# li779/mitsuba-im

Hardware: AMD Instinct MI355X
Metric: Msamples/sec at 1920x1080 path-trace, max depth 8 (higher is better)
Workload: dtype f32; 1 GPU; C2: Cornell box (synthetic, 32 triangles), 1920x1080, sobol sampler, 256 spp (256 per GPU-share), maxDepth 8, rrDepth 5, box filter, 1xMI355X wavefront path tracer per GPU; one process per GPU, rows interleaved over the ranks, RCCL film reduce; parallelism=tiles1, face=C-ABI (mi_render_run)

## Files before the change

### mitsuba-im_amd/csrc/kernels_trace.hip

```cpp
#include "kernels_common.h"
#include <algorithm>
#include "trace.h"
#include "trace_fused.h"

template <int STACK, int AN, bool WIDE>
__global__ __launch_bounds__(WG) void k_extend(DScene sc, Queues q, int buf) {
    __shared__ int s_stk[(STACK > 0 ? STACK : 1) * WG];
    __shared__ f4 s_exact[STACK > 0 ? 1 : MI_PACKET_MAX * 3];
    const uint32_t tid = threadIdx.x;
    unsigned long long rays = 0;
    if (STACK == 0) packetStage(sc, s_exact);
    for (uint32_t seg = blockIdx.x; seg < q.n_seg; seg += gridDim.x) {
    const uint32_t n = q.count[buf][seg];
    const uint64_t segBase = (uint64_t) seg * q.cap;
    rays += n;
    for (uint32_t i = tid; i < n; i += WG) {
        float4 ro = q.rayO[buf][segBase + i], rd = q.rayD[buf][segBase + i];
        v3 o = V(ro.x, ro.y, ro.z), d = V(rd.x, rd.y, rd.z);
        float mint, maxt, t = 0, u = 0, v = 0; uint32_t prim = 0xFFFFFFFFu; bool hit = false; int inst = -1;
        if (clipInterval(sc, o, d, ro.w, rd.w, false, mint, maxt)) {
            if (STACK == 0) hit = packetIntersect<false, AN>(sc, (AS<true>::p4) s_exact, o, d, mint, maxt, t, prim, u, v);
            else hit = traverse<false, AN, WIDE>(sc, o, d, mint, maxt, s_stk + tid, t, prim, u, v, inst);
        }
        q.hit[segBase + i] = make_float4(t, u, v, __uint_as_float(hit ? prim : 0xFFFFFFFFu));
        if ((AN & 2) && q.hitInst) q.hitInst[segBase + i] = inst;
    }
    }
    if (tid == 0 && rays) atomicAdd(&q.counters[0], rays);
}

template <int STACK, int AN, bool WIDE>
__global__ __launch_bounds__(WG) void k_shadow(DScene sc, Queues q) {
    __shared__ int s_stk[(STACK > 0 ? STACK : 1) * WG];
    __shared__ f4 s_exact[STACK > 0 ? 1 : MI_PACKET_MAX * 3];
    const uint32_t tid = threadIdx.x;
    if (STACK == 0) packetStage(sc, s_exact);
    for (uint32_t seg = blockIdx.x; seg < q.n_seg; seg += gridDim.x) {
    const uint32_t n = q.shCount[seg];
    const uint64_t segBase = (uint64_t) seg * q.cap;
    for (uint32_t i = tid; i < n; i += WG) {
        float4 so = q.shO[segBase + i], sd = q.shD[segBase + i];
        v3 o = V(so.x, so.y, so.z), d = V(sd.x, sd.y, sd.z);
        float mint, maxt, t, u, v; uint32_t prim; bool occluded = false; int inst;
        if (clipInterval(sc, o, d, MI_EPSILON, so.w, true, mint, maxt)) {
            if (STACK == 0) occluded = packetIntersect<true, AN>(sc, (AS<true>::p4) s_exact, o, d, mint, maxt, t, prim, u, v);
            else occluded = traverse<true, AN, WIDE>(sc, o, d, mint, maxt, s_stk + tid, t, prim, u, v, inst);
        }
        if (!occluded) {
            float4 c = q.shC[segBase + i]; const uint32_t pid = __float_as_uint(sd.w);
            float4 a = q.acc[pid]; a.x += c.x; a.y += c.y; a.z += c.z; q.acc[pid] = a;
        }
    }
    }
}



template <bool WIDE>
__global__ __launch_bounds__(WG) void k_extend_f(DScene sc, Queues q, int buf, uint32_t *ticket, uint32_t thr) {
    __shared__ int s_lds[FZ_LDS_WORDS];
    fusedStage<false, WIDE>(sc, q, buf, ticket, thr, s_lds);
}
template <bool WIDE>
__global__ __launch_bounds__(WG) void k_shadow_f(DScene sc, Queues q, uint32_t *ticket, uint32_t thr) {
    __shared__ int s_lds[FZ_LDS_WORDS];
    fusedStage<true, WIDE>(sc, q, 0, ticket, thr, s_lds);
}

template <bool ANY, bool WIDE, int LS>
__global__ __launch_bounds__(WG) void k_debug_fused(DScene sc, Queues q, uint32_t *ticket, uint32_t thr, int *maxSp) {
    __shared__ int s_lds[(LS + 10) * WG];
    fusedStage<ANY, WIDE, LS, true>(sc, q, 0, ticket, thr, s_lds, maxSp);
}

__global__ __launch_bounds__(WG) void k_debug_intersect(DScene sc, const float *rays, uint64_t n, int anyHit, float *out, int *outInst) {
    __shared__ int s_stk[STACK_DEPTH * WG];
    __shared__ f4 s_exact[MI_PACKET_MAX * 3];
    if (sc.packet_n) packetStage(sc, s_exact);
    const uint64_t i = (uint64_t) blockIdx.x * WG + threadIdx.x;
    if (i >= n) return;
    const float *r = rays + i * 8;
    v3 o = V(r[0], r[1], r[2]), d = V(r[4], r[5], r[6]);
    float mint, maxt, t = 0, u = 0, v = 0; uint32_t prim = 0xFFFFFFFFu; bool hit = false; int inst = -1;
    if (clipInterval(sc, o, d, r[3], r[7], anyHit != 0, mint, maxt)) {
        if (sc.packet_n) { if (anyHit) hit = packetIntersect<true, 1>(sc, (AS<true>::p4) s_exact, o, d, mint, maxt, t, prim, u, v); else hit = packetIntersect<false, 1>(sc, (AS<true>::p4) s_exact, o, d, mint, maxt, t, prim, u, v); }
        else if (sc.bvh_wide) { if (anyHit) hit = traverse<true, 3, true>(sc, o, d, mint, maxt, s_stk + threadIdx.x, t, prim, u, v, inst); else hit = traverse<false, 3, true>(sc, o, d, mint, maxt, s_stk + threadIdx.x, t, prim, u, v, inst); }
        else if (anyHit) hit = traverse<true, 3, false>(sc, o, d, mint, maxt, s_stk + threadIdx.x, t, prim, u, v, inst);
        else hit = traverse<false, 3, false>(sc, o, d, mint, maxt, s_stk + threadIdx.x, t, prim, u, v, inst);
    }
    if (outInst) outInst[i] = hit ? inst : -1;
    out[i * 4] = t; out[i * 4 + 1] = u; out[i * 4 + 2] = v; out[i * 4 + 3] = hit ? (anyHit ? 1.0f : (float) prim) : -1.0f;
}

__global__ __launch_bounds__(WG) void k_ray_intersect(DScene sc, const float *rays, uint64_t n, mi_intersection *out) {
    __shared__ int s_stk[STACK_DEPTH * WG];
    __shared__ f4 s_exact[MI_PACKET_MAX * 3];
    if (sc.packet_n) packetStage(sc, s_exact);
    const uint64_t i = (uint64_t) blockIdx.x * WG + threadIdx.x;
    if (i >= n) return;
    const float *r = rays + i * 8;
    v3 o = V(r[0], r[1], r[2]), d = V(r[4], r[5], r[6]);
    float mint, maxt, t = 0, u = 0, v = 0; uint32_t prim = 0xFFFFFFFFu; bool hit = false; int inst = -1;
    if (clipInterval(sc, o, d, r[3], r[7], false, mint, maxt)) {
        if (sc.packet_n) hit = packetIntersect<false, 1>(sc, (AS<true>::p4) s_exact, o, d, mint, maxt, t, prim, u, v);
        else if (sc.bvh_wide) hit = traverse<false, 3, true>(sc, o, d, mint, maxt, s_stk + threadIdx.x, t, prim, u, v, inst);
        else hit = traverse<false, 3, false>(sc, o, d, mint, maxt, s_stk + threadIdx.x, t, prim, u, v, inst);
    }
    mi_intersection rec; memset(&rec, 0, sizeof(rec)); rec.valid = hit ? 1u : 0u; rec.prim = 0xFFFFFFFFu; rec.instance = -1; rec.material = -1; rec.emitter = -1;
    if (hit) {
        Tabs<false> tb; tb.shade4 = (AS<false>::p4) sc.shade; tb.materials4 = (AS<false>::p4) sc.materials; tb.emitters4 = (AS<false>::p4) sc.emitters; tb.emitter_cdf = sc.emitter_cdf; tb.area_cdf = sc.area_cdf;
        Hit h;
        if (inst >= 0) fillHitInstanced(sc, tb, sc.instances[inst], o, d, t, prim, u, v, h);
        else if (prim >= sc.n_tris) fillHitAnalytic(sc.analytic[prim - sc.n_tris], o, d, t, u, v, h);
        else fillHit<false, true>(sc, tb, d, t, prim, u, v, h);
        if (inst < 0 && prim >= sc.n_tris) { v3 du, dv; analyticUV(sc.analytic[prim - sc.n_tris], u, v, o + d * t, h.uvx, h.uvy, du, dv); }
        rec.t = t; rec.p[0] = h.p.x; rec.p[1] = h.p.y; rec.p[2] = h.p.z; rec.ng[0] = h.ng.x; rec.ng[1] = h.ng.y; rec.ng[2] = h.ng.z;
        rec.ns[0] = h.ns.x; rec.ns[1] = h.ns.y; rec.ns[2] = h.ns.z; rec.s[0] = h.s.x; rec.s[1] = h.s.y; rec.s[2] = h.s.z; rec.tt[0] = h.t.x; rec.tt[1] = h.t.y; rec.tt[2] = h.t.z;
        rec.uv[0] = h.uvx; rec.uv[1] = h.uvy; rec.wi[0] = h.wi.x; rec.wi[1] = h.wi.y; rec.wi[2] = h.wi.z; rec.bary[0] = u; rec.bary[1] = v;
        rec.prim = prim; rec.instance = inst; rec.material = h.material; rec.emitter = h.emitter;
    }
    out[i] = rec;
}

extern "C" {
static const bool kForceStack24 = getenv("MI355PT_STACK24") != nullptr;
#define MI_BY_STACK_W(KERNEL, AN, W, ...) do { \
    if (sc.bvh_depth <= 8) hipLaunchKernelGGL((KERNEL<8, AN, W>), dim3(grid), dim3(WG), 0, st, __VA_ARGS__); \
    else if (sc.bvh_depth <= 12) hipLaunchKernelGGL((KERNEL<12, AN, W>), dim3(grid), dim3(WG), 0, st, __VA_ARGS__); \
    else if (sc.bvh_depth <= 16) hipLaunchKernelGGL((KERNEL<16, AN, W>), dim3(grid), dim3(WG), 0, st, __VA_ARGS__); \
    else if (sc.bvh_depth <= 20 && !kForceStack24) hipLaunchKernelGGL((KERNEL<20, AN, W>), dim3(grid), dim3(WG), 0, st, __VA_ARGS__); \
    else if (sc.bvh_depth <= 24) hipLaunchKernelGGL((KERNEL<24, AN, W>), dim3(grid), dim3(WG), 0, st, __VA_ARGS__); \
    else if (sc.bvh_depth <= 28) hipLaunchKernelGGL((KERNEL<28, AN, W>), dim3(grid), dim3(WG), 0, st, __VA_ARGS__); \
    else hipLaunchKernelGGL((KERNEL<STACK_DEPTH, AN, W>), dim3(grid), dim3(WG), 0, st, __VA_ARGS__); } while (0)
#define MI_BY_STACK(KERNEL, AN, ...) do { \
    if (sc.packet_n) hipLaunchKernelGGL((KERNEL<0, (AN) & 1, false>), dim3(grid), dim3(WG), 0, st, __VA_ARGS__); \
    else if (sc.bvh_wide) MI_BY_STACK_W(KERNEL, AN, true, __VA_ARGS__); \
    else MI_BY_STACK_W(KERNEL, AN, false, __VA_ARGS__); } while (0)
void mi_launch_extend(const DScene &sc, const Queues &q, int buf, uint32_t grid, hipStream_t st) {
    const int mode = (sc.n_analytic ? 1 : 0) | (sc.n_instances ? 2 : 0);
    if (mode == 3) MI_BY_STACK(k_extend, 3, sc, q, buf); else if (mode == 2) MI_BY_STACK(k_extend, 2, sc, q, buf); else if (mode == 1) MI_BY_STACK(k_extend, 1, sc, q, buf); else MI_BY_STACK(k_extend, 0, sc, q, buf);
}
void mi_launch_shadow(const DScene &sc, const Queues &q, uint32_t grid, hipStream_t st) {
    const int mode = (sc.n_analytic ? 1 : 0) | (sc.n_instances ? 2 : 0);
    if (mode == 3) MI_BY_STACK(k_shadow, 3, sc, q); else if (mode == 2) MI_BY_STACK(k_shadow, 2, sc, q); else if (mode == 1) MI_BY_STACK(k_shadow, 1, sc, q); else MI_BY_STACK(k_shadow, 0, sc, q);
}
#undef MI_BY_STACK
#undef MI_BY_STACK_W
static const int kFused = [] { const char *e = getenv("MI355PT_FUSED"); return e && e[0] ? atoi(e) : 1; }();
static const uint32_t kFusedThr = [] { const char *e = getenv("MI355PT_FUSED_THR"); const int v = e && e[0] ? atoi(e) : 48; return (uint32_t) (v < 1 ? 1 : (v > 64 ? 64 : v)); }();
static const uint32_t kFusedGrid = [] { const char *e = getenv("MI355PT_FUSED_GRID"); const int v = e && e[0] ? atoi(e) : 1792; return (uint32_t) (v < 1 ? 1 : (v > 16384 ? 16384 : v)); }();
bool mi_fused_walk(const DScene &sc) { return kFused && (sc.bvh_wide || kFused == 2) && !sc.packet_n && !sc.n_analytic && !sc.n_instances && sc.geo_bytes < 0xFFFFFF00ull; }
uint32_t mi_fused_grid(void) { return kFusedGrid; }
void mi_launch_extend_fused(const DScene &sc, const Queues &q, int buf, uint32_t *ticket, hipStream_t st) {
    const uint32_t g = kFusedGrid;
    if (sc.bvh_wide) hipLaunchKernelGGL((k_extend_f<true>), dim3(g), dim3(WG), 0, st, sc, q, buf, ticket, kFusedThr); else hipLaunchKernelGGL((k_extend_f<false>), dim3(g), dim3(WG), 0, st, sc, q, buf, ticket, kFusedThr);
}
void mi_launch_shadow_fused(const DScene &sc, const Queues &q, uint32_t *ticket, hipStream_t st) {
    const uint32_t g = kFusedGrid;
    if (sc.bvh_wide) hipLaunchKernelGGL((k_shadow_f<true>), dim3(g), dim3(WG), 0, st, sc, q, ticket, kFusedThr); else hipLaunchKernelGGL((k_shadow_f<false>), dim3(g), dim3(WG), 0, st, sc, q, ticket, kFusedThr);
}
void mi_launch_debug_fused(const DScene &sc, const Queues &q, int anyHit, uint32_t ldsStack, uint32_t *ticket, uint32_t thr, uint32_t grid, int *maxSp, hipStream_t st) {
#define MI_DBG_FUSED(ANY, WIDE) do { \
    if (ldsStack == 4u) hipLaunchKernelGGL((k_debug_fused<ANY, WIDE, 4>), dim3(grid), dim3(WG), 0, st, sc, q, ticket, thr, maxSp); \
    else hipLaunchKernelGGL((k_debug_fused<ANY, WIDE, FZ_LDS_STACK>), dim3(grid), dim3(WG), 0, st, sc, q, ticket, thr, maxSp); } while (0)
    if (anyHit) { if (sc.bvh_wide) MI_DBG_FUSED(true, true); else MI_DBG_FUSED(true, false); }
    else { if (sc.bvh_wide) MI_DBG_FUSED(false, true); else MI_DBG_FUSED(false, false); }
#undef MI_DBG_FUSED
}
uint32_t mi_fused_lds_stack(void) { return FZ_LDS_STACK; }
void mi_launch_ray_intersect(const DScene &sc, const float *rays, uint64_t n, mi_intersection *out, hipStream_t st) { hipLaunchKernelGGL(k_ray_intersect, dim3((unsigned) ((n + WG - 1) / WG)), dim3(WG), 0, st, sc, rays, n, out); }
void mi_launch_debug_intersect(const DScene &sc, const float *rays, uint64_t n, int anyHit, float *out, int *outInst, hipStream_t st) { hipLaunchKernelGGL(k_debug_intersect, dim3((unsigned) ((n + WG - 1) / WG)), dim3(WG), 0, st, sc, rays, n, anyHit, out, outInst); }
}
```

### mitsuba-im_amd/csrc/scene_build.cpp

```cpp
#include "scene_host.h"
#include <algorithm>
#include <cmath>
#include <cstdlib>
#include <cstring>
#include <limits>

namespace mi {

struct V3 { float x, y, z; };
static inline V3 mk(float x, float y, float z) { return V3{x, y, z}; }
static inline V3 operator+(V3 a, V3 b) { return mk(a.x + b.x, a.y + b.y, a.z + b.z); }
static inline V3 operator-(V3 a, V3 b) { return mk(a.x - b.x, a.y - b.y, a.z - b.z); }
static inline V3 operator*(V3 a, float s) { return mk(a.x * s, a.y * s, a.z * s); }
static inline float dot(V3 a, V3 b) { return a.x * b.x + a.y * b.y + a.z * b.z; }
static inline V3 cross(V3 a, V3 b) { return mk(a.y * b.z - a.z * b.y, a.z * b.x - a.x * b.z, a.x * b.y - a.y * b.x); }
static inline float comp(V3 a, int i) { return i == 0 ? a.x : (i == 1 ? a.y : a.z); }
static inline V3 normalize(V3 a) { float inv = 1.0f / std::sqrt(dot(a, a)); return a * inv; }
static inline V3 vmin(V3 a, V3 b) { return mk(std::min(a.x, b.x), std::min(a.y, b.y), std::min(a.z, b.z)); }
static inline V3 vmax(V3 a, V3 b) { return mk(std::max(a.x, b.x), std::max(a.y, b.y), std::max(a.z, b.z)); }

static void triaccelLoad(TriAccelD &ta, V3 A, V3 B, V3 C) {
    static const int wald[4] = {1, 2, 0, 1};
    V3 b = C - A, c = B - A, N = cross(c, b);
    int k = 0;
// ... 301 lines not shown
                            int ql = (int) std::floor(((double) comp(k.lo, a) - o) / step), qh = (int) std::ceil(((double) comp(k.hi, a) - o) / step);
                            ql = std::min(std::max(ql, 0), 255); qh = std::min(std::max(qh, 0), 255);
                            while (ql > 0 && (float) ((float) o + (float) ql * (float) step) > comp(k.lo, a)) --ql;
                            while (qh < 255 && (float) ((float) o + (float) qh * (float) step) < comp(k.hi, a)) ++qh;
                            w.qlo[a] |= (uint32_t) ql << (8 * c); w.qhi[a] |= (uint32_t) qh << (8 * c);
                        }
                        if (k.count > 0) w.child[c] = leafCode(triBase + k.first, k.count);
                        else { int need = 0, needD = 0; w.child[c] = run(kids[c], need, needD); sub = std::max(sub, need); subD = std::max(subD, needD); }
                    }
                    std::memcpy(&nodes[dev], &w, sizeof(w));
                    need = sub + 1;
                    needD = subD + 3;
                    return dev;
                } };
            Emit em{nodes, bld, triBase, emptyChild, area}; int need = 0, needD = 0; const int dev = em.run(root, need, needD); treeNeed.push_back(need + 1); treeNeedDirect.push_back(needD + 1);
            (void) nodeBase; return dev;
        }
        std::vector<int> devIndex(bld.nodes.size(), -1); int nInner = 0;
        for (size_t i = 0; i < bld.nodes.size(); ++i) if (bld.nodes[i].count == 0) devIndex[i] = nodeBase + nInner++;
        auto childCode = [&](int c) { const BuildNode &n = bld.nodes[c]; return n.count > 0 ? leafCode(triBase + n.first, n.count) : (int32_t) devIndex[c]; };
        if (root < 0) { BvhNode n{}; emptyBox(n.lo0, n.hi0); emptyBox(n.lo1, n.hi1); n.c0 = n.c1 = leafCode(0, 1); nodes.push_back(n); return nodeBase; }
        if (bld.nodes[root].count > 0) {
            BvhNode n{}; setBox(n.lo0, n.hi0, bld.nodes[root]); n.c0 = leafCode(triBase + bld.nodes[root].first, bld.nodes[root].count);
            emptyBox(n.lo1, n.hi1); n.c1 = n.c0; nodes.push_back(n); return nodeBase;
        }
        nodes.resize(nodeBase + nInner);
        for (size_t i = 0; i < bld.nodes.size(); ++i) {
            const BuildNode &b = bld.nodes[i]; if (b.count > 0) continue;
            BvhNode &n = nodes[devIndex[i]]; std::memset(&n, 0, sizeof(n));
            setBox(n.lo0, n.hi0, bld.nodes[b.left]); setBox(n.lo1, n.hi1, bld.nodes[b.right]);
            n.c0 = childCode(b.left); n.c1 = childCode(b.right);
        }
        return devIndex[root];
    };
    std::vector<std::vector<uint32_t> > members(ng + 1);
    for (const mi_shape &sh : shapes) { uint32_t g = slotOf(sh); for (uint32_t t = 0; t < sh.tri_count; ++t) members[g].push_back(sh.first_tri + t); }
    for (uint32_t t = nt; t < np; ++t) members[ng].push_back(t);
    emitTree(members[ng]);
    if (wideBvh && ni == 0 && ng == 0 && nodes.size() > 1) {
        Bvh4Node *w = reinterpret_cast<Bvh4Node *>(nodes.data()); const size_t nn = nodes.size();
        std::vector<float> areaOf(nn, 0.0f); areaOf[0] = std::numeric_limits<float>::infinity();
        for (size_t i = 0; i < nn; ++i) for (int c = 0; c < 4; ++c) if (w[i].child[c] >= 0) {
            const float st[3] = {w[i].step_x, w[i].step_y, w[i].step_z}; float e[3];
            for (int a = 0; a < 3; ++a) e[a] = (float) ((int) ((w[i].qhi[a] >> (8 * c)) & 0xFFu) - (int) ((w[i].qlo[a] >> (8 * c)) & 0xFFu)) * st[a];
            areaOf[w[i].child[c]] = e[0] * e[1] + e[1] * e[2] + e[2] * e[0];
        }
        std::vector<uint32_t> byArea(nn); for (size_t i = 0; i < nn; ++i) byArea[i] = (uint32_t) i;
        std::stable_sort(byArea.begin(), byArea.end(), [&](uint32_t a, uint32_t b) { return areaOf[a] > areaOf[b]; });
        std::vector<int32_t> newIndex(nn); for (size_t i = 0; i < nn; ++i) newIndex[byArea[i]] = (int32_t) i;
        std::vector<BvhNode> re(nn);
        for (size_t i = 0; i < nn; ++i) {
            Bvh4Node n = w[byArea[i]];
            for (int c = 0; c < 4; ++c) if (n.child[c] >= 0) n.child[c] = newIndex[n.child[c]];
            std::memcpy(&re[i], &n, sizeof(n));
        }
        nodes.swap(re);
    }
    std::vector<int> groupRoot(ng, 0);
    for (uint32_t g = 0; g < ng; ++g) groupRoot[g] = emitTree(members[g]);
    for (uint32_t i = 0; i < ni; ++i) instancesD[i].root = groupRoot[instances[i].group];
    if (wideBvh) {
        int groupNeed = 0; for (uint32_t g = 0; g < ng; ++g) groupNeed = std::max(groupNeed, treeNeed[1 + g]);
        bvhDepth = treeNeed[0] + (ni ? 1 + groupNeed : 0);
        bvhStackDirect = treeNeedDirect[0];
    } else {
        struct Depth { const std::vector<BvhNode> &n; int of(int i) const { if (i < 0) return 0; int a = of(n[i].c0), b = of(n[i].c1); return 1 + (a > b ? a : b); } } dep{nodes};
        int groupDepth = 0; for (uint32_t g = 0; g < ng; ++g) groupDepth = std::max(groupDepth, dep.of(groupRoot[g]));
        bvhDepth = dep.of(0) + (ni ? 1 + groupDepth : 0);
        bvhStackDirect = dep.of(0);
    }
    packetExact.assign(accel.begin(), accel.begin() + nt); packetGroups.clear(); packetGK[0] = packetGK[1] = packetGK[2] = 0;
    {
        float sx = 0; for (int i = 0; i < 3; ++i) sx = std::max(sx, std::max(std::fabs(aabbLo[i]), std::fabs(aabbHi[i])));
        packetScale = sx;
        if (nt <= MI_PACKET_MAX && ni == 0) {
            const float tol = 1e-6f * std::max(sx, 1e-20f);
            auto near = [&](V3 a, V3 b) { return std::fabs(a.x - b.x) <= tol && std::fabs(a.y - b.y) <= tol && std::fabs(a.z - b.z) <= tol; };
            std::vector<uint8_t> used(nt, 0); std::vector<PacketGroupD> byAxis[3];
            for (uint32_t t1 = 0; t1 < nt; ++t1) {
                if (used[t1] || accel[t1].k > 2) continue;
                used[t1] = 1;
                const V3 P[3] = {vert(idx[t1 * 3]), vert(idx[t1 * 3 + 1]), vert(idx[t1 * 3 + 2])};
                int partner = -1, rot = 0;
                for (uint32_t t2 = t1 + 1; t2 < nt && partner < 0; ++t2) {
                    if (used[t2] || accel[t2].k != accel[t1].k) continue;
                    const V3 Q[3] = {vert(idx[t2 * 3]), vert(idx[t2 * 3 + 1]), vert(idx[t2 * 3 + 2])};
                    for (int r = 0; r < 3 && partner < 0; ++r) {
                        const V3 X = P[r], Y = P[(r + 1) % 3], Z = P[(r + 2) % 3], X2 = Y + Z - X;
                        for (int a = 0; a < 3 && partner < 0; ++a)
                            for (int b = 0; b < 3 && partner < 0; ++b) { if (b == a) continue; const int c = 3 - a - b;
                                if (near(Q[a], Y) && near(Q[b], Z) && near(Q[c], X2)) { partner = (int) t2; rot = r; } }
                    }
                }
                const V3 X = P[rot], Y = P[(rot + 1) % 3], Z = P[(rot + 2) % 3];
                TriAccelD ta; triaccelLoad(ta, partner >= 0 ? Z : P[0], partner >= 0 ? X : P[1], partner >= 0 ? Y : P[2]);
                if (ta.k > 2) continue;
                if (partner >= 0) used[partner] = 1;
                PacketGroupD g; g.n_u = ta.n_u; g.n_v = ta.n_v; g.n_d = ta.n_d; g.a_u = ta.a_u; g.a_v = ta.a_v; g.b_nu = ta.b_nu; g.b_nv = ta.b_nv; g.c_nu = ta.c_nu; g.c_nv = ta.c_nv;
                g.margin = 1.1f * (std::fabs(ta.b_nu) + std::fabs(ta.b_nv) + std::fabs(ta.c_nu) + std::fabs(ta.c_nv));
                g.prim0 = t1; g.prim1 = partner >= 0 ? (uint32_t) partner : 0xFFFFFFFFu;
                byAxis[ta.k].push_back(g);
            }
            for (int axis = 0; axis < 3; ++axis) { packetGroups.insert(packetGroups.end(), byAxis[axis].begin(), byAxis[axis].end()); packetGK[axis] = (uint32_t) packetGroups.size(); }
        }
    }
    if (packetGroups.empty()) packetGroups.push_back(PacketGroupD{});
    if (packetExact.empty()) packetExact.push_back(TriAccelD{});

    const uint32_t ne = (uint32_t) emitters.size();
    emitterCdf.assign(ne + 1, 0.0f); emittersD.assign(ne, EmitterD{}); areaCdf.clear(); emitterNorm = 0.0f;
    emitterX.assign((size_t) std::max(ne, 1u) * 16, 0.0f); hasDeltaEmitters = false;
    for (uint32_t e = 0; e < ne; ++e) emitterCdf[e + 1] = emitterCdf[e] + emitters[e].weight;
    if (ne) { float sum = emitterCdf[ne]; emitterNorm = sum > 0 ? 1.0f / sum : 0.0f; for (uint32_t e = 1; e <= ne; ++e) emitterCdf[e] *= emitterNorm; emitterCdf[ne] = 1.0f; }
    for (uint32_t e = 0; e < ne; ++e) {
        EmitterD &d = emittersD[e]; const mi_emitter &src = emitters[e];
        d.radiance[0] = src.radiance[0]; d.radiance[1] = src.radiance[1]; d.radiance[2] = src.radiance[2]; d.weight = src.weight;
        d.type = src.type; d.shape = src.shape;
        d.analytic = -1;
        float *x = &emitterX[e * 16];
        if (src.type == MI_EMITTER_POINT || src.type == MI_EMITTER_SPOT) { x[0] = src.to_world[3]; x[1] = src.to_world[7]; x[2] = src.to_world[11]; hasDeltaEmitters = true; }
        if (src.type == MI_EMITTER_COLLIMATED) { x[0] = src.to_world[3]; x[1] = src.to_world[7]; x[2] = src.to_world[11]; hasDeltaEmitters = true; }
        if (src.type == MI_EMITTER_DIRECTIONAL) { x[0] = src.to_world[2]; x[1] = src.to_world[6]; x[2] = src.to_world[10]; hasDeltaEmitters = true; }
        if (src.type == MI_EMITTER_SPOT) {
            float beam = src.beam * (MI_PI / 180.0f), cutoff = src.cutoff * (MI_PI / 180.0f);
            x[13] = std::cos(beam); x[3] = std::cos(cutoff); x[14] = cutoff; x[15] = 1.0f / (cutoff - beam);
            const float *m = src.to_world; float *o = x + 4;
            float a[9] = {m[0], m[1], m[2], m[4], m[5], m[6], m[8], m[9], m[10]};
            float det = a[0] * (a[4] * a[8] - a[5] * a[7]) - a[1] * (a[3] * a[8] - a[5] * a[6]) + a[2] * (a[3] * a[7] - a[4] * a[6]); float id = 1.0f / det;
            o[0] = (a[4] * a[8] - a[5] * a[7]) * id; o[1] = (a[2] * a[7] - a[1] * a[8]) * id; o[2] = (a[1] * a[5] - a[2] * a[4]) * id;
            o[3] = (a[5] * a[6] - a[3] * a[8]) * id; o[4] = (a[0] * a[8] - a[2] * a[6]) * id; o[5] = (a[2] * a[3] - a[0] * a[5]) * id;
            o[6] = (a[3] * a[7] - a[4] * a[6]) * id; o[7] = (a[1] * a[6] - a[0] * a[7]) * id; o[8] = (a[0] * a[4] - a[1] * a[3]) * id;
        }
        if (src.type != MI_EMITTER_AREA) continue;
        if ((size_t) src.shape >= shapes.size()) {
            d.analytic = src.shape - (int32_t) shapes.size(); d.inv_area = analyticD[d.analytic].inv_area; continue;
        }
        const mi_shape &sh = shapes[src.shape];
        d.first_tri = sh.first_tri; d.tri_count = sh.tri_count; d.cdf_offset = (uint32_t) areaCdf.size();
        size_t base = areaCdf.size(); areaCdf.resize(base + sh.tri_count + 1); areaCdf[base] = 0.0f;
        for (uint32_t t = 0; t < sh.tri_count; ++t) {
            uint32_t prim = sh.first_tri + t;
            V3 p0 = vert(idx[prim * 3]), p1 = vert(idx[prim * 3 + 1]), p2 = vert(idx[prim * 3 + 2]);
            V3 c = cross(p1 - p0, p2 - p0);
            areaCdf[base + t + 1] = areaCdf[base + t] + 0.5f * std::sqrt(dot(c, c));
        }
        float sum = areaCdf[base + sh.tri_count], norm = 1.0f / sum;
        for (uint32_t t = 1; t <= sh.tri_count; ++t) areaCdf[base + t] *= norm;
        areaCdf[base + sh.tri_count] = 1.0f;
        d.inv_area = 1.0f / sum;
    }
    if (areaCdf.empty()) areaCdf.push_back(0.0f);

    {
        const uint32_t kind = filterKind;
        float radius = kind == 0 ? filterRadius + 1e-5f : kind == 1 ? 4.0f * filterStddev : kind == 2 ? 1.0f : kind == 5 ? (float) (int) filterRadius : 2.0f;
        float alpha = -1.0f / (2.0f * filterStddev * filterStddev), bias = std::exp(alpha * radius * radius);
        const float B = kind == 3 ? filterRadius : 0.0f, C = kind == 3 ? filterStddev : 0.5f;
        float sum = 0.0f;
        for (int i = 0; i < MI_FILTER_RES; ++i) {
            float x = (radius * (float) i) / (float) MI_FILTER_RES, v;
            if (kind == 0) v = std::fabs(x) <= radius ? 1.0f : 0.0f;
            else if (kind == 1) v = std::max(0.0f, std::exp(alpha * x * x) - bias);
            else if (kind == 2) v = std::max(0.0f, 1.0f - std::fabs(x / radius));
            else if (kind == 5) {
                float ax = std::fabs(x);
                if (ax < 1e-4f) v = 1.0f; else if (ax > radius) v = 0.0f;
                else { float x1 = MI_PI * ax, x2 = x1 / radius; v = (std::sin(x1) * std::sin(x2)) / (x1 * x2); }
            } else {
                float ax = std::fabs(x), x2 = ax * ax, x3 = x2 * ax;
                if (ax < 1) v = 1.0f / 6.0f * ((12 - 9 * B - 6 * C) * x3 + (-18 + 12 * B + 6 * C) * x2 + (6 - 2 * B));
                else if (ax < 2) v = 1.0f / 6.0f * ((-B - 6 * C) * x3 + (6 * B + 30 * C) * x2 + (-12 * B - 48 * C) * ax + (8 * B + 24 * C));
                else v = 0.0f;
            }
            filterValues[i] = v; sum += v;
        }
        filterValues[MI_FILTER_RES] = 0.0f;
        filterScale = (float) MI_FILTER_RES / radius; filterRadiusEff = radius;
        border = (int) std::ceil(radius - 0.5f);
        sum *= 2 * radius / (float) MI_FILTER_RES;
        float norm = 1.0f / sum;
        for (int i = 0; i < MI_FILTER_RES; ++i) filterValues[i] *= norm;
    }
    envIndex = -1; envConstant = false;
// ... 52 lines not shown
```

### mitsuba-im_amd/csrc/trace.h

```cpp
#pragma once
#include "kernels_common.h"

DEV bool slab(f4 lo, f4 hi, v3 inv, v3 oi, float tmin, float tmax, float &tnear) {
    float ax = __builtin_fmaf(lo.x, inv.x, oi.x), bx = __builtin_fmaf(hi.x, inv.x, oi.x);
    float ay = __builtin_fmaf(lo.y, inv.y, oi.y), by = __builtin_fmaf(hi.y, inv.y, oi.y);
    float az = __builtin_fmaf(lo.z, inv.z, oi.z), bz = __builtin_fmaf(hi.z, inv.z, oi.z);
    float t0 = fmaxf(fmaxf(fminf(ax, bx), fminf(ay, by)), fmaxf(fminf(az, bz), tmin));
    float t1 = fminf(fminf(fmaxf(ax, bx), fmaxf(ay, by)), fminf(fmaxf(az, bz), tmax));
    tnear = t0;
    return t0 <= t1 * 1.000002f + 1e-30f;
}
DEV bool aabbRay(const float *lo, const float *hi, v3 o, v3 d, float &nearT, float &farT) {
    float nt = -INFINITY, ft = INFINITY;
    const float oo[3] = {o.x, o.y, o.z}, dd[3] = {d.x, d.y, d.z};
#pragma unroll
    for (int i = 0; i < 3; ++i) {
        float origin = oo[i], minv = lo[i], maxv = hi[i], di = dd[i];
        if (di == 0) { if (origin < minv || origin > maxv) return false; }
        else {
            float rcp = 1.0f / di;
            float t1 = (minv - origin) * rcp, t2 = (maxv - origin) * rcp;
            if (t1 > t2) { float tmp = t1; t1 = t2; t2 = tmp; }
            nt = maxf(t1, nt); ft = minf(t2, ft);
            if (!(nt <= ft)) return false;
// ... 38 lines not shown
                const uint32_t lx = __float_as_uint(n1.x), ly = __float_as_uint(n1.y), lz = __float_as_uint(n1.z), hx = __float_as_uint(n1.w), hy = __float_as_uint(n2.x), hz = __float_as_uint(n2.y);
                const uint32_t nxq = inv.x >= 0 ? lx : hx, fxq = inv.x >= 0 ? hx : lx, nyq = inv.y >= 0 ? ly : hy, fyq = inv.y >= 0 ? hy : ly, nzq = inv.z >= 0 ? lz : hz, fzq = inv.z >= 0 ? hz : lz;
                const float far = (AN & 2) ? fminf(best, cap) : best;
                uint32_t key[4];
#pragma unroll
                for (int c = 0; c < 4; ++c) {
                    const float tn = fmaxf(fmaxf(__builtin_fmaf((float) ((nxq >> (8 * c)) & 0xFFu), bx, ax), __builtin_fmaf((float) ((nyq >> (8 * c)) & 0xFFu), by, ay)),
                                           fmaxf(__builtin_fmaf((float) ((nzq >> (8 * c)) & 0xFFu), bz, az), mint));
                    const float tf = fminf(fminf(__builtin_fmaf((float) ((fxq >> (8 * c)) & 0xFFu), bx, ax), __builtin_fmaf((float) ((fyq >> (8 * c)) & 0xFFu), by, ay)),
                                           fminf(__builtin_fmaf((float) ((fzq >> (8 * c)) & 0xFFu), bz, az), far));
                    key[c] = (tn <= tf * 1.000002f + 1e-30f) ? ((__float_as_uint(tn) & ~3u) | (uint32_t) c) : 0xFFFFFFFFu;
                }
                {
                    uint32_t a = min(key[0], key[1]), b = max(key[0], key[1]), c = min(key[2], key[3]), e = max(key[2], key[3]);
                    key[0] = min(a, c); const uint32_t m1 = max(a, c), m2 = min(b, e); key[3] = max(b, e); key[1] = min(m1, m2); key[2] = max(m1, m2);
                }
                const int c0 = __float_as_int(n3.x), c1 = __float_as_int(n3.y), c2 = __float_as_int(n3.z), c3 = __float_as_int(n3.w);
                auto childOf = [&](uint32_t k) { const uint32_t sl = k & 3u; return sl == 0u ? c0 : (sl == 1u ? c1 : (sl == 2u ? c2 : c3)); };
                if (key[0] == 0xFFFFFFFFu) BVH_POP();
                else {
                    const uint32_t more = (key[1] != 0xFFFFFFFFu) + (key[2] != 0xFFFFFFFFu) + (key[3] != 0xFFFFFFFFu);
                    if (more) { stk[sp * WG] = (int) ((uint32_t) cur | ((key[1] & 3u) << 23) | ((key[2] & 3u) << 25) | ((key[3] & 3u) << 27) | ((more - 1u) << 29)); ++sp; }
                    cur = childOf(key[0]);
                }
            }
        } else
        while (cur >= 0 && cur != BVH_DONE) {
            f4 n0 = nodes4[cur * 4 + 0], n1 = nodes4[cur * 4 + 1], n2 = nodes4[cur * 4 + 2], n3 = nodes4[cur * 4 + 3];
            int c0 = __float_as_int(n0.w), c1 = __float_as_int(n1.w);
            float t0, t1;
            const float far = (AN & 2) ? fminf(best, cap) : best;
            bool h0 = slab(n0, n1, inv, oi, mint, far, t0), h1 = slab(n2, n3, inv, oi, mint, far, t1);
            if (h0 && h1) {
                bool swap = t1 < t0;
                stk[sp * WG] = swap ? c0 : c1; ++sp;
                cur = swap ? c1 : c0;
            } else if (h0) cur = c0;
            else if (h1) cur = c1;
            else BVH_POP();
        }
        if (cur == BVH_DONE) break;
        {
            uint32_t code = (uint32_t) ~cur; uint32_t first = code >> 3, cnt = (code & 7u) + 1u;
            bool entered = false;
            for (uint32_t i = 0; i < cnt; ++i) {
                f4 a = tris4[(first + i) * 3 + 0], b = tris4[(first + i) * 3 + 1], c = tris4[(first + i) * 3 + 2];
                TriAccelD ta; ta.k = __float_as_uint(a.x); ta.n_u = a.y; ta.n_v = a.z; ta.n_d = a.w;
                ta.a_u = b.x; ta.a_v = b.y; ta.b_nu = b.z; ta.b_nv = b.w; ta.c_nu = c.x; ta.c_nv = c.y; ta.prim = __float_as_uint(c.z);
                float u, v, t; bool ok;
                if ((AN & 2) && ta.k == MI_K_INSTANCE) {
                    const InstanceD &in = sc.instances[ta.prim];
                    v3 o2 = xfPoint(in.to_object, o0), d2 = xfVector(in.to_object, d0);
                    float nearT, farT;
                    if (aabbRay(in.glo, in.ghi, o2, d2, nearT, farT)) {
                        const float mi = mint0 > nearT ? mint0 : nearT, ma = best < farT ? best : farT;
                        if (ma > mi) {
                            stk[sp * WG] = BVH_RET; ++sp;
                            o = o2; d = d2; mint = mi; cap = farT; curInst = (int) ta.prim;
                            inv = V(safeInv(d.x), safeInv(d.y), safeInv(d.z)); oi = V(-o.x * inv.x, -o.y * inv.y, -o.z * inv.z);
                            cur = in.root; entered = true;
                        }
                    }
                    break;
                }
                const float far = (AN & 2) ? fminf(best, cap) : best;
                if ((AN & 1) && ta.k == MI_K_ANALYTIC) ok = analyticIntersect<ANY>(sc.analytic[ta.prim - sc.n_tris], o, d, mint, far, t, u, v);
                else ok = triIntersect(ta, o, d, mint, far, u, v, t);
                if (ok) {
                    if (ANY) return true;
                    if (!found || t < best || (t == best && (ta.prim < bprim || (ta.prim == bprim && curInst < binst)))) { best = t; bprim = ta.prim; binst = curInst; bu = u; bv = v; found = true; }
                }
            }
            if (!entered) BVH_POP();
        }
    }
#undef BVH_POP
    bestT = best; bestPrim = bprim; bestU = bu; bestV = bv; bestInst = binst;
    return found;
}

typedef const __attribute__((address_space(4))) f4 *cf4p;
struct PacketGroupS { f4 g0, g1, g2; };
typedef const __attribute__((address_space(4))) PacketGroupS *cgrp;
template <typename MaskT> DEV MaskT maskBit(uint32_t p) { return p < sizeof(MaskT) * 8u ? (MaskT) 1 << p : (MaskT) 0; }
template <int K, typename MaskT>
DEV void packetPass1(cgrp g, uint32_t count, v3 o, v3 d, float mint, float maxt, float so1e5, MaskT &mask) {
    const float o_u = K == 0 ? o.y : (K == 1 ? o.z : o.x), o_v = K == 0 ? o.z : (K == 1 ? o.x : o.y), o_k = K == 0 ? o.x : (K == 1 ? o.y : o.z);
    const float d_u = K == 0 ? d.y : (K == 1 ? d.z : d.x), d_v = K == 0 ? d.z : (K == 1 ? d.x : d.y), d_k = K == 0 ? d.x : (K == 1 ? d.y : d.z);
    for (; count; --count, ++g) {
        const f4 g0 = g->g0, g1 = g->g1, g2 = g->g2;
        const MaskT bit0 = maskBit<MaskT>(__float_as_uint(g2.z)), bit1 = maskBit<MaskT>(__float_as_uint(g2.w));
        const float D = __builtin_fmaf(d_u, g0.x, __builtin_fmaf(d_v, g0.y, d_k));
        const float N = __builtin_fmaf(-o_v, g0.y, __builtin_fmaf(-o_u, g0.x, g0.z - o_k));
        const float r = __builtin_amdgcn_rcpf(D), t = N * r, q = fabsf(r) + 1.0f;
        const float mt = q * __builtin_fmaf(fabsf(t), 2e-6f, so1e5);
        const float hu = __builtin_fmaf(t, d_u, o_u - g0.w), hv = __builtin_fmaf(t, d_v, o_v - g1.x);
        const float u = __builtin_fmaf(hv, g1.y, hu * g1.z), v = __builtin_fmaf(hu, g1.w, hv * g2.x);
        const float m = g2.y * mt, s = u + v, one = 1.0f + m;
        const bool reject = (fabsf(D) >= 1e-4f) & ((t + mt < mint) | (t - mt > maxt) | (s < -m) | (s > one) | (v < -m) | (v > one));
        mask |= (reject | (u < -m)) ? (MaskT) 0 : bit0;
        mask |= (reject | (u > m)) ? (MaskT) 0 : bit1;
    }
}
template <bool ANY, int AN, typename MaskT>
DEV bool packetIntersectM(const DScene &sc, AS<true>::p4 s_exact, v3 o, v3 d, float mint, float maxt, float &bestT, uint32_t &bestPrim, float &bestU, float &bestV) {
    float best = maxt; uint32_t bprim = 0xFFFFFFFFu; bool found = false; float bu = 0, bv = 0;
    MaskT mask = 0;
    const float so1e5 = maxf(maxf(sc.packet_scale, fabsf(o.x)), maxf(fabsf(o.y), fabsf(o.z))) * 1e-5f;
    cgrp groups = (cgrp) sc.packet_groups;
    packetPass1<0, MaskT>(groups, sc.packet_gk[0], o, d, mint, maxt, so1e5, mask);
    packetPass1<1, MaskT>(groups + sc.packet_gk[0], sc.packet_gk[1] - sc.packet_gk[0], o, d, mint, maxt, so1e5, mask);
    packetPass1<2, MaskT>(groups + sc.packet_gk[1], sc.packet_gk[2] - sc.packet_gk[1], o, d, mint, maxt, so1e5, mask);
    while (mask) {
        const uint32_t i = sizeof(MaskT) == 8 ? (uint32_t) __builtin_ctzll((unsigned long long) mask) : (uint32_t) __builtin_ctz((uint32_t) mask); mask &= mask - 1;
        const f4 a = s_exact[i * 3u], b = s_exact[i * 3u + 1u], c = s_exact[i * 3u + 2u];
        const bool k0 = __float_as_uint(a.x) == 0u, k1 = __float_as_uint(a.x) == 1u;
        const float o_u = k0 ? o.y : (k1 ? o.z : o.x), o_v = k0 ? o.z : (k1 ? o.x : o.y), o_k = k0 ? o.x : (k1 ? o.y : o.z);
        const float d_u = k0 ? d.y : (k1 ? d.z : d.x), d_v = k0 ? d.z : (k1 ? d.x : d.y), d_k = k0 ? d.x : (k1 ? d.y : d.z);
        const float tt = (a.w - o_u * a.y - o_v * a.z - o_k) / (d_u * a.y + d_v * a.z + d_k);
        const float hu = o_u + tt * d_u - b.x, hv = o_v + tt * d_v - b.y;
        const float uu = hv * b.z + hu * b.w, vv = hu * c.x + hv * c.y;
        const bool ok = !(tt < mint) & !(tt > best) & (uu >= 0) & (vv >= 0) & (uu + vv <= 1.0f);
        if (ANY) { found |= ok; mask = ok ? (MaskT) 0 : mask; }
        else {
            const bool better = ok & (!found | (tt < best));
            best = better ? tt : best; bprim = better ? i : bprim; bu = better ? uu : bu; bv = better ? vv : bv; found |= ok;
        }
    }
    if (ANY && found) return true;
    if (AN & 1) {
        for (uint32_t i = 0; i < sc.n_analytic; ++i) {
            AnalyticD sh;
            { cf4p src = (cf4p) (sc.analytic + i); f4 *dst = reinterpret_cast<f4 *>(&sh);
#pragma unroll
              for (int j = 0; j < 10; ++j) dst[j] = src[j]; }
            float u, v, t; const uint32_t prim = sc.n_tris + i;
            if (analyticIntersect<ANY>(sh, o, d, mint, best, t, u, v)) {
                if (ANY) return true;
                if (!found || t < best || prim < bprim) { best = t; bprim = prim; bu = u; bv = v; found = true; }
            }
        }
    }
    bestT = best; bestPrim = bprim; bestU = bu; bestV = bv;
    return found;
}
template <bool ANY, int AN>
DEV bool packetIntersect(const DScene &sc, AS<true>::p4 s_exact, v3 o, v3 d, float mint, float maxt, float &bestT, uint32_t &bestPrim, float &bestU, float &bestV) {
    if (sc.n_tris <= 32u) return packetIntersectM<ANY, AN, uint32_t>(sc, s_exact, o, d, mint, maxt, bestT, bestPrim, bestU, bestV);
    return packetIntersectM<ANY, AN, unsigned long long>(sc, s_exact, o, d, mint, maxt, bestT, bestPrim, bestU, bestV);
}
DEV void packetStage(const DScene &sc, f4 *s_exact) {
    const f4 *src = reinterpret_cast<const f4 *>(sc.packet_exact);
    for (uint32_t i = threadIdx.x; i < sc.n_tris * 3u; i += blockDim.x) s_exact[i] = src[i];
    __syncthreads();
}
```

Before: 3217 Msamples/s.

## Software-pipeline packet group loads and index ray components via LDS

Rewrites the packet-pass loop so it double-buffers the scalar group loads with sched barriers, overlapping the next group's fetch with the current test. Replaces the two per-bit mask computations with a single shifted 2-bit OR that uses a paired flag. Stores each ray's rotated origin and direction in per-thread LDS so the exact-test stage indexes them by axis instead of using select chains. It also limits triangle pairing to adjacent triangles so prim1 is implicit, which can reduce pairing in other scenes. It adds an optional debug step histogram, raises LDS usage per block, and costs extra LDS writes on every ray.

```diff
diff --git a/mitsuba-im_amd/csrc/kernels_trace.hip b/mitsuba-im_amd/csrc/kernels_trace.hip
--- a/mitsuba-im_amd/csrc/kernels_trace.hip
+++ b/mitsuba-im_amd/csrc/kernels_trace.hip
@@ -6,10 +6,10 @@
 template <int STACK, int AN, bool WIDE>
 __global__ __launch_bounds__(WG) void k_extend(DScene sc, Queues q, int buf) {
     __shared__ int s_stk[(STACK > 0 ? STACK : 1) * WG];
-    __shared__ f4 s_exact[STACK > 0 ? 1 : MI_PACKET_MAX * 3];
+    __shared__ f4 s_packet[STACK > 0 ? 1 : PK_LDS_F4];
     const uint32_t tid = threadIdx.x;
     unsigned long long rays = 0;
-    if (STACK == 0) packetStage(sc, s_exact);
+    PacketLds pk{}; if (STACK == 0) pk = packetStage(sc, s_packet);
     for (uint32_t seg = blockIdx.x; seg < q.n_seg; seg += gridDim.x) {
     const uint32_t n = q.count[buf][seg];
     const uint64_t segBase = (uint64_t) seg * q.cap;
@@ -19,7 +19,7 @@
         v3 o = V(ro.x, ro.y, ro.z), d = V(rd.x, rd.y, rd.z);
         float mint, maxt, t = 0, u = 0, v = 0; uint32_t prim = 0xFFFFFFFFu; bool hit = false; int inst = -1;
         if (clipInterval(sc, o, d, ro.w, rd.w, false, mint, maxt)) {
-            if (STACK == 0) hit = packetIntersect<false, AN>(sc, (AS<true>::p4) s_exact, o, d, mint, maxt, t, prim, u, v);
+            if (STACK == 0) hit = packetIntersect<false, AN>(sc, pk, o, d, mint, maxt, t, prim, u, v);
             else hit = traverse<false, AN, WIDE>(sc, o, d, mint, maxt, s_stk + tid, t, prim, u, v, inst);
         }
         q.hit[segBase + i] = make_float4(t, u, v, __uint_as_float(hit ? prim : 0xFFFFFFFFu));
@@ -32,9 +32,9 @@
 template <int STACK, int AN, bool WIDE>
 __global__ __launch_bounds__(WG) void k_shadow(DScene sc, Queues q) {
     __shared__ int s_stk[(STACK > 0 ? STACK : 1) * WG];
-    __shared__ f4 s_exact[STACK > 0 ? 1 : MI_PACKET_MAX * 3];
+    __shared__ f4 s_packet[STACK > 0 ? 1 : PK_LDS_F4];
     const uint32_t tid = threadIdx.x;
-    if (STACK == 0) packetStage(sc, s_exact);
+    PacketLds pk{}; if (STACK == 0) pk = packetStage(sc, s_packet);
     for (uint32_t seg = blockIdx.x; seg < q.n_seg; seg += gridDim.x) {
     const uint32_t n = q.shCount[seg];
     const uint64_t segBase = (uint64_t) seg * q.cap;
@@ -43,7 +43,7 @@
         v3 o = V(so.x, so.y, so.z), d = V(sd.x, sd.y, sd.z);
         float mint, maxt, t, u, v; uint32_t prim; bool occluded = false; int inst;
         if (clipInterval(sc, o, d, MI_EPSILON, so.w, true, mint, maxt)) {
-            if (STACK == 0) occluded = packetIntersect<true, AN>(sc, (AS<true>::p4) s_exact, o, d, mint, maxt, t, prim, u, v);
+            if (STACK == 0) occluded = packetIntersect<true, AN>(sc, pk, o, d, mint, maxt, t, prim, u, v);
             else occluded = traverse<true, AN, WIDE>(sc, o, d, mint, maxt, s_stk + tid, t, prim, u, v, inst);
         }
         if (!occluded) {
@@ -75,15 +75,15 @@
 
 __global__ __launch_bounds__(WG) void k_debug_intersect(DScene sc, const float *rays, uint64_t n, int anyHit, float *out, int *outInst) {
     __shared__ int s_stk[STACK_DEPTH * WG];
-    __shared__ f4 s_exact[MI_PACKET_MAX * 3];
-    if (sc.packet_n) packetStage(sc, s_exact);
+    __shared__ f4 s_packet[PK_LDS_F4];
+    PacketLds pk{}; if (sc.packet_n) pk = packetStage(sc, s_packet);
     const uint64_t i = (uint64_t) blockIdx.x * WG + threadIdx.x;
     if (i >= n) return;
     const float *r = rays + i * 8;
     v3 o = V(r[0], r[1], r[2]), d = V(r[4], r[5], r[6]);
     float mint, maxt, t = 0, u = 0, v = 0; uint32_t prim = 0xFFFFFFFFu; bool hit = false; int inst = -1;
     if (clipInterval(sc, o, d, r[3], r[7], anyHit != 0, mint, maxt)) {
-        if (sc.packet_n) { if (anyHit) hit = packetIntersect<true, 1>(sc, (AS<true>::p4) s_exact, o, d, mint, maxt, t, prim, u, v); else hit = packetIntersect<false, 1>(sc, (AS<true>::p4) s_exact, o, d, mint, maxt, t, prim, u, v); }
+        if (sc.packet_n) { if (anyHit) hit = packetIntersect<true, 1>(sc, pk, o, d, mint, maxt, t, prim, u, v); else hit = packetIntersect<false, 1>(sc, pk, o, d, mint, maxt, t, prim, u, v); }
         else if (sc.bvh_wide) { if (anyHit) hit = traverse<true, 3, true>(sc, o, d, mint, maxt, s_stk + threadIdx.x, t, prim, u, v, inst); else hit = traverse<false, 3, true>(sc, o, d, mint, maxt, s_stk + threadIdx.x, t, prim, u, v, inst); }
         else if (anyHit) hit = traverse<true, 3, false>(sc, o, d, mint, maxt, s_stk + threadIdx.x, t, prim, u, v, inst);
         else hit = traverse<false, 3, false>(sc, o, d, mint, maxt, s_stk + threadIdx.x, t, prim, u, v, inst);
@@ -94,15 +94,15 @@
 
 __global__ __launch_bounds__(WG) void k_ray_intersect(DScene sc, const float *rays, uint64_t n, mi_intersection *out) {
     __shared__ int s_stk[STACK_DEPTH * WG];
-    __shared__ f4 s_exact[MI_PACKET_MAX * 3];
-    if (sc.packet_n) packetStage(sc, s_exact);
+    __shared__ f4 s_packet[PK_LDS_F4];
+    PacketLds pk{}; if (sc.packet_n) pk = packetStage(sc, s_packet);
     const uint64_t i = (uint64_t) blockIdx.x * WG + threadIdx.x;
     if (i >= n) return;
     const float *r = rays + i * 8;
     v3 o = V(r[0], r[1], r[2]), d = V(r[4], r[5], r[6]);
     float mint, maxt, t = 0, u = 0, v = 0; uint32_t prim = 0xFFFFFFFFu; bool hit = false; int inst = -1;
     if (clipInterval(sc, o, d, r[3], r[7], false, mint, maxt)) {
-        if (sc.packet_n) hit = packetIntersect<false, 1>(sc, (AS<true>::p4) s_exact, o, d, mint, maxt, t, prim, u, v);
+        if (sc.packet_n) hit = packetIntersect<false, 1>(sc, pk, o, d, mint, maxt, t, prim, u, v);
         else if (sc.bvh_wide) hit = traverse<false, 3, true>(sc, o, d, mint, maxt, s_stk + threadIdx.x, t, prim, u, v, inst);
         else hit = traverse<false, 3, false>(sc, o, d, mint, maxt, s_stk + threadIdx.x, t, prim, u, v, inst);
     }
@@ -168,6 +168,13 @@
 #undef MI_DBG_FUSED
 }
 uint32_t mi_fused_lds_stack(void) { return FZ_LDS_STACK; }
+#ifdef MI_PACKET_STEP_HIST
+int mi_debug_packet_steps(unsigned long long *out) {
+    unsigned long long zero[2][36] = {};
+    if (hipDeviceSynchronize() != hipSuccess || hipMemcpyFromSymbol(out, HIP_SYMBOL(g_packetSteps), sizeof(zero)) != hipSuccess) return 1;
+    return hipMemcpyToSymbol(HIP_SYMBOL(g_packetSteps), zero, sizeof(zero)) != hipSuccess;
+}
+#endif
 void mi_launch_ray_intersect(const DScene &sc, const float *rays, uint64_t n, mi_intersection *out, hipStream_t st) { hipLaunchKernelGGL(k_ray_intersect, dim3((unsigned) ((n + WG - 1) / WG)), dim3(WG), 0, st, sc, rays, n, out); }
 void mi_launch_debug_intersect(const DScene &sc, const float *rays, uint64_t n, int anyHit, float *out, int *outInst, hipStream_t st) { hipLaunchKernelGGL(k_debug_intersect, dim3((unsigned) ((n + WG - 1) / WG)), dim3(WG), 0, st, sc, rays, n, anyHit, out, outInst); }
 }
diff --git a/mitsuba-im_amd/csrc/scene_build.cpp b/mitsuba-im_amd/csrc/scene_build.cpp
--- a/mitsuba-im_amd/csrc/scene_build.cpp
+++ b/mitsuba-im_amd/csrc/scene_build.cpp
@@ -407,8 +407,8 @@
                 used[t1] = 1;
                 const V3 P[3] = {vert(idx[t1 * 3]), vert(idx[t1 * 3 + 1]), vert(idx[t1 * 3 + 2])};
                 int partner = -1, rot = 0;
-                for (uint32_t t2 = t1 + 1; t2 < nt && partner < 0; ++t2) {
-                    if (used[t2] || accel[t2].k != accel[t1].k) continue;
+                if (t1 + 1 < nt && !used[t1 + 1] && accel[t1 + 1].k == accel[t1].k) {
+                    const uint32_t t2 = t1 + 1;
                     const V3 Q[3] = {vert(idx[t2 * 3]), vert(idx[t2 * 3 + 1]), vert(idx[t2 * 3 + 2])};
                     for (int r = 0; r < 3 && partner < 0; ++r) {
                         const V3 X = P[r], Y = P[(r + 1) % 3], Z = P[(r + 2) % 3], X2 = Y + Z - X;
@@ -423,7 +423,7 @@
                 if (partner >= 0) used[partner] = 1;
                 PacketGroupD g; g.n_u = ta.n_u; g.n_v = ta.n_v; g.n_d = ta.n_d; g.a_u = ta.a_u; g.a_v = ta.a_v; g.b_nu = ta.b_nu; g.b_nv = ta.b_nv; g.c_nu = ta.c_nu; g.c_nv = ta.c_nv;
                 g.margin = 1.1f * (std::fabs(ta.b_nu) + std::fabs(ta.b_nv) + std::fabs(ta.c_nu) + std::fabs(ta.c_nv));
-                g.prim0 = t1; g.prim1 = partner >= 0 ? (uint32_t) partner : 0xFFFFFFFFu;
+                g.prim0 = t1; g.prim1 = partner >= 0 ? t1 + 1u : 0xFFFFFFFFu;
                 byAxis[ta.k].push_back(g);
             }
             for (int axis = 0; axis < 3; ++axis) { packetGroups.insert(packetGroups.end(), byAxis[axis].begin(), byAxis[axis].end()); packetGK[axis] = (uint32_t) packetGroups.size(); }
diff --git a/mitsuba-im_amd/csrc/trace.h b/mitsuba-im_amd/csrc/trace.h
--- a/mitsuba-im_amd/csrc/trace.h
+++ b/mitsuba-im_amd/csrc/trace.h
@@ -144,41 +144,73 @@
 typedef const __attribute__((address_space(4))) f4 *cf4p;
 struct PacketGroupS { f4 g0, g1, g2; };
 typedef const __attribute__((address_space(4))) PacketGroupS *cgrp;
-template <typename MaskT> DEV MaskT maskBit(uint32_t p) { return p < sizeof(MaskT) * 8u ? (MaskT) 1 << p : (MaskT) 0; }
+#define PK_RAY_WORDS 10
+#define PK_LDS_F4 (MI_PACKET_MAX * 3 + PK_RAY_WORDS * WG / 4)
+typedef __attribute__((address_space(3))) float *ldsf;
+struct PacketLds { AS<true>::p4 exact; ldsf ray; };
+#ifdef MI_PACKET_STEP_HIST
+static __device__ unsigned long long g_packetSteps[2][36];
+DEV uint32_t pkWaveMax(uint32_t v) { for (int s = 32; s; s >>= 1) { const uint32_t w = (uint32_t) __shfl_xor((int) v, s, 64); v = w > v ? w : v; } return v; }
+DEV uint32_t pkWaveSum(uint32_t v) { for (int s = 32; s; s >>= 1) v += (uint32_t) __shfl_xor((int) v, s, 64); return v; }
+#endif
+DEV PacketGroupS packetLoad(cgrp p) { PacketGroupS r; r.g0 = p->g0; r.g1 = p->g1; r.g2 = p->g2; return r; }
+template <typename MaskT>
+DEV void packetTest1(const PacketGroupS &G, float o_u, float o_v, float o_k, float d_u, float d_v, float d_k, float mint, float maxt, float so1e5, MaskT &mask) {
+    const f4 g0 = G.g0, g1 = G.g1, g2 = G.g2;
+    const float D = __builtin_fmaf(d_u, g0.x, __builtin_fmaf(d_v, g0.y, d_k));
+    const float N = __builtin_fmaf(-o_v, g0.y, __builtin_fmaf(-o_u, g0.x, g0.z - o_k));
+    const float r = __builtin_amdgcn_rcpf(D), t = N * r, q = fabsf(r) + 1.0f;
+    const float mt = q * __builtin_fmaf(fabsf(t), 2e-6f, so1e5);
+    const float hu = __builtin_fmaf(t, d_u, o_u - g0.w), hv = __builtin_fmaf(t, d_v, o_v - g1.x);
+    const float u = __builtin_fmaf(hv, g1.y, hu * g1.z), v = __builtin_fmaf(hu, g1.w, hv * g2.x);
+    const float m = g2.y * mt, s = u + v, one = 1.0f + m;
+    const bool reject = (fabsf(D) >= 1e-4f) & ((t + mt < mint) | (t - mt > maxt) | (s < -m) | (s > one) | (v < -m) | (v > one));
+    const bool paired = __float_as_uint(g2.w) != 0xFFFFFFFFu;
+    const bool c0 = !(reject | (u < -m)), c1 = !(reject | (u > m)) & paired;
+    const uint32_t x = (c1 ? 2u : 0u) | (c0 ? 1u : 0u);
+    mask |= (MaskT) x << __float_as_uint(g2.z);
+}
+#define PK_ARRIVED(R) asm volatile("" :: "s"((R).g0.x), "s"((R).g2.w))
 template <int K, typename MaskT>
 DEV void packetPass1(cgrp g, uint32_t count, v3 o, v3 d, float mint, float maxt, float so1e5, MaskT &mask) {
     const float o_u = K == 0 ? o.y : (K == 1 ? o.z : o.x), o_v = K == 0 ? o.z : (K == 1 ? o.x : o.y), o_k = K == 0 ? o.x : (K == 1 ? o.y : o.z);
     const float d_u = K == 0 ? d.y : (K == 1 ? d.z : d.x), d_v = K == 0 ? d.z : (K == 1 ? d.x : d.y), d_k = K == 0 ? d.x : (K == 1 ? d.y : d.z);
-    for (; count; --count, ++g) {
-        const f4 g0 = g->g0, g1 = g->g1, g2 = g->g2;
-        const MaskT bit0 = maskBit<MaskT>(__float_as_uint(g2.z)), bit1 = maskBit<MaskT>(__float_as_uint(g2.w));
-        const float D = __builtin_fmaf(d_u, g0.x, __builtin_fmaf(d_v, g0.y, d_k));
-        const float N = __builtin_fmaf(-o_v, g0.y, __builtin_fmaf(-o_u, g0.x, g0.z - o_k));
-        const float r = __builtin_amdgcn_rcpf(D), t = N * r, q = fabsf(r) + 1.0f;
-        const float mt = q * __builtin_fmaf(fabsf(t), 2e-6f, so1e5);
-        const float hu = __builtin_fmaf(t, d_u, o_u - g0.w), hv = __builtin_fmaf(t, d_v, o_v - g1.x);
-        const float u = __builtin_fmaf(hv, g1.y, hu * g1.z), v = __builtin_fmaf(hu, g1.w, hv * g2.x);
-        const float m = g2.y * mt, s = u + v, one = 1.0f + m;
-        const bool reject = (fabsf(D) >= 1e-4f) & ((t + mt < mint) | (t - mt > maxt) | (s < -m) | (s > one) | (v < -m) | (v > one));
-        mask |= (reject | (u < -m)) ? (MaskT) 0 : bit0;
-        mask |= (reject | (u > m)) ? (MaskT) 0 : bit1;
-    }
-}
+    const uint32_t n = (uint32_t) __builtin_amdgcn_readfirstlane((int) count);
+    if (n == 0u) return;
+    const uint32_t last = n - 1u;
+    PacketGroupS A = packetLoad(g);
+    uint32_t i = 0;
+    for (; i < last; i += 2u) {
+        PK_ARRIVED(A);
+        const PacketGroupS B = packetLoad(g + (i + 1u)); __builtin_amdgcn_sched_barrier(0);
+        packetTest1<MaskT>(A, o_u, o_v, o_k, d_u, d_v, d_k, mint, maxt, so1e5, mask);
+        PK_ARRIVED(B);
+        A = packetLoad(g + (i + 2u < last ? i + 2u : last)); __builtin_amdgcn_sched_barrier(0);
+        packetTest1<MaskT>(B, o_u, o_v, o_k, d_u, d_v, d_k, mint, maxt, so1e5, mask);
+    }
+    if (i == last) packetTest1<MaskT>(A, o_u, o_v, o_k, d_u, d_v, d_k, mint, maxt, so1e5, mask);
+}
+#undef PK_ARRIVED
 template <bool ANY, int AN, typename MaskT>
-DEV bool packetIntersectM(const DScene &sc, AS<true>::p4 s_exact, v3 o, v3 d, float mint, float maxt, float &bestT, uint32_t &bestPrim, float &bestU, float &bestV) {
+DEV bool packetIntersectM(const DScene &sc, const PacketLds &lds, v3 o, v3 d, float mint, float maxt, float &bestT, uint32_t &bestPrim, float &bestU, float &bestV) {
     float best = maxt; uint32_t bprim = 0xFFFFFFFFu; bool found = false; float bu = 0, bv = 0;
     MaskT mask = 0;
+    const ldsf ray = lds.ray;
+    ray[0] = o.x; ray[WG] = o.y; ray[2 * WG] = o.z; ray[3 * WG] = o.x; ray[4 * WG] = o.y;
+    ray[5 * WG] = d.x; ray[6 * WG] = d.y; ray[7 * WG] = d.z; ray[8 * WG] = d.x; ray[9 * WG] = d.y;
     const float so1e5 = maxf(maxf(sc.packet_scale, fabsf(o.x)), maxf(fabsf(o.y), fabsf(o.z))) * 1e-5f;
     cgrp groups = (cgrp) sc.packet_groups;
     packetPass1<0, MaskT>(groups, sc.packet_gk[0], o, d, mint, maxt, so1e5, mask);
     packetPass1<1, MaskT>(groups + sc.packet_gk[0], sc.packet_gk[1] - sc.packet_gk[0], o, d, mint, maxt, so1e5, mask);
     packetPass1<2, MaskT>(groups + sc.packet_gk[1], sc.packet_gk[2] - sc.packet_gk[1], o, d, mint, maxt, so1e5, mask);
+#ifdef MI_PACKET_STEP_HIST
+    uint32_t dbgSteps = 0; const uint32_t dbgCand = sizeof(MaskT) == 8 ? (uint32_t) __builtin_popcountll((unsigned long long) mask) : (uint32_t) __builtin_popcount((uint32_t) mask);
+#endif
     while (mask) {
         const uint32_t i = sizeof(MaskT) == 8 ? (uint32_t) __builtin_ctzll((unsigned long long) mask) : (uint32_t) __builtin_ctz((uint32_t) mask); mask &= mask - 1;
-        const f4 a = s_exact[i * 3u], b = s_exact[i * 3u + 1u], c = s_exact[i * 3u + 2u];
-        const bool k0 = __float_as_uint(a.x) == 0u, k1 = __float_as_uint(a.x) == 1u;
-        const float o_u = k0 ? o.y : (k1 ? o.z : o.x), o_v = k0 ? o.z : (k1 ? o.x : o.y), o_k = k0 ? o.x : (k1 ? o.y : o.z);
-        const float d_u = k0 ? d.y : (k1 ? d.z : d.x), d_v = k0 ? d.z : (k1 ? d.x : d.y), d_k = k0 ? d.x : (k1 ? d.y : d.z);
+        const f4 a = lds.exact[i * 3u], b = lds.exact[i * 3u + 1u], c = lds.exact[i * 3u + 2u];
+        const ldsf rk = ray + __float_as_uint(a.x) * WG;
+        const float o_k = rk[0], o_u = rk[WG], o_v = rk[2 * WG], d_k = rk[5 * WG], d_u = rk[6 * WG], d_v = rk[7 * WG];
         const float tt = (a.w - o_u * a.y - o_v * a.z - o_k) / (d_u * a.y + d_v * a.z + d_k);
         const float hu = o_u + tt * d_u - b.x, hv = o_v + tt * d_v - b.y;
         const float uu = hv * b.z + hu * b.w, vv = hu * c.x + hv * c.y;
@@ -188,7 +220,15 @@
             const bool better = ok & (!found | (tt < best));
             best = better ? tt : best; bprim = better ? i : bprim; bu = better ? uu : bu; bv = better ? vv : bv; found |= ok;
         }
-    }
+#ifdef MI_PACKET_STEP_HIST
+        ++dbgSteps;
+#endif
+    }
+#ifdef MI_PACKET_STEP_HIST
+    {   const uint32_t wmax = pkWaveMax(dbgSteps), wsum = pkWaveSum(dbgCand), lanes = (uint32_t) __popcll(__ballot(1));
+        if ((uint32_t) (__ffsll((long long) __ballot(1)) - 1) == (threadIdx.x & 63u)) {
+            atomicAdd(&g_packetSteps[ANY ? 1 : 0][wmax < 33u ? wmax : 33u], 1ull); atomicAdd(&g_packetSteps[ANY ? 1 : 0][34], (unsigned long long) wsum); atomicAdd(&g_packetSteps[ANY ? 1 : 0][35], (unsigned long long) lanes); } }
+#endif
     if (ANY && found) return true;
     if (AN & 1) {
         for (uint32_t i = 0; i < sc.n_analytic; ++i) {
@@ -207,12 +247,14 @@
     return found;
 }
 template <bool ANY, int AN>
-DEV bool packetIntersect(const DScene &sc, AS<true>::p4 s_exact, v3 o, v3 d, float mint, float maxt, float &bestT, uint32_t &bestPrim, float &bestU, float &bestV) {
-    if (sc.n_tris <= 32u) return packetIntersectM<ANY, AN, uint32_t>(sc, s_exact, o, d, mint, maxt, bestT, bestPrim, bestU, bestV);
-    return packetIntersectM<ANY, AN, unsigned long long>(sc, s_exact, o, d, mint, maxt, bestT, bestPrim, bestU, bestV);
-}
-DEV void packetStage(const DScene &sc, f4 *s_exact) {
+DEV bool packetIntersect(const DScene &sc, const PacketLds &lds, v3 o, v3 d, float mint, float maxt, float &bestT, uint32_t &bestPrim, float &bestU, float &bestV) {
+    if (sc.n_tris <= 32u) return packetIntersectM<ANY, AN, uint32_t>(sc, lds, o, d, mint, maxt, bestT, bestPrim, bestU, bestV);
+    return packetIntersectM<ANY, AN, unsigned long long>(sc, lds, o, d, mint, maxt, bestT, bestPrim, bestU, bestV);
+}
+DEV PacketLds packetStage(const DScene &sc, f4 *s_packet) {
     const f4 *src = reinterpret_cast<const f4 *>(sc.packet_exact);
-    for (uint32_t i = threadIdx.x; i < sc.n_tris * 3u; i += blockDim.x) s_exact[i] = src[i];
+    for (uint32_t i = threadIdx.x; i < sc.n_tris * 3u; i += blockDim.x) s_packet[i] = src[i];
     __syncthreads();
-}
+    PacketLds lds; lds.exact = (AS<true>::p4) s_packet; lds.ray = (ldsf) reinterpret_cast<float *>(s_packet + MI_PACKET_MAX * 3) + threadIdx.x;
+    return lds;
+}
```

Result: faster. 3313 Msamples/s, median of 6 (+3.0%).
